# marios2019/CSN

Measured on AMD Instinct MI355X. Metric: CSA fwd+bwd points/sec (10k pts x 256 ch, K=3), higher is better.
Workload: dtype bf16x3 (fp32 operands split into 2 bf16, 3 bf16 MFMA per product, fp32 accumulate); 1 GPU; BASELINE configs[2]: CSA K=3, 32 query shapes/GPU x 10000 pts x 256 ch, n_heads=1, d_k=d_v=256, 20 blocks of 500, 39 classes, fwd + masked CE + bwd, train mode (dropout 0.1 live, 2K+2 evaluations/shape), math mode bf16x3; K=3, parallelism=single GPU

## Files before the change

### csn_amd/_lib.py

```python
from __future__ import annotations

import ctypes
import hashlib
import os
import subprocess
from ctypes import c_char_p, c_double, c_float, c_int, c_longlong, c_ulonglong, c_void_p
from typing import Optional

_HERE = os.path.dirname(os.path.abspath(__file__))
_CSRC = os.path.join(_HERE, "csrc")
LIB_PATH = os.path.join(_HERE, "libcsn_hip.so")
SOURCES = ["gemm_f32.hip", "gemm_bf16x3.hip", "wx_stream.hip", "wx_lnb.hip", "loss.hip", "attn_f32.hip", "attn_bf16x3.hip", "attn_dkv.hip", "attn_dv_scores.hip", "fold.hip", "outproj_ln.hip", "retrieval.hip", "retrieval_screen.hip", "combine.hip", "compat.hip", "minkowski_csn.hip", "minkowski_seg.hip", "rows_fc.hip", "sparse_conv.hip", "sparse_conv_maps16.hip", "train_maps16.hip", "sparse_conv_cat.hip", "octant_conv.hip", "octant_conv_maps16.hip", "octant_conv_stats.hip", "rows_bn_act.hip", "point_field.hip", "kernel_map.hip", "octant_map.hip", "points.hip", "csn_capi.hip"]
HEADERS = ["csn_common.h", "csn_kernels.h", "csn_window.h", "attn_tile_image.h", "wx_common.h", "rows_mma.h", "sconv_gemm_body.inc", "sconv_a16_body.inc", "rows_bn_act_body.inc", "octant_rows_body.inc", os.path.join("..", "..", "include", "csn_hip.h")]
ARCH = "gfx950"
BUILD_FLAGS = [f"--offload-arch={ARCH}", "-O3", "-std=c++17", "-fPIC", "-fvisibility=hidden", "-shared"]

_lib: Optional[ctypes.CDLL] = None


class CsnError(RuntimeError):
    pass


class BnTerms(ctypes.Structure):
# ... 285 lines not shown
    "csn_sparse_conv_stats_fwd_t16": (c_int, [c_void_p, c_int, c_longlong, c_int, c_void_p, c_int, c_int, c_int, c_int, c_void_p, c_void_p,
                                              c_longlong, c_void_p, c_void_p, c_void_p, c_void_p, c_float, c_float, c_void_p,
                                              c_longlong, c_void_p]),
    "csn_rows_bn_act_fwd_t16": (c_int, [c_void_p, c_int, c_int, c_int, c_int, c_float, c_void_p, c_int, c_longlong, c_int, c_void_p,
                                        c_int, c_longlong, c_void_p]),
    "csn_rows_bn_act_bwd_t16": (c_int, [c_void_p, c_longlong, c_void_p, c_int, c_longlong, c_void_p, c_int, c_int, c_int, c_int,
                                        c_float, c_int, c_void_p, c_longlong, c_void_p, c_longlong, c_void_p]),
    "csn_sparse_conv_bwd_t16": (c_int, [c_void_p, c_longlong, c_void_p, c_int, c_longlong, c_int, c_int, c_int, c_int, c_int, c_void_p,
                                        c_void_p, c_void_p, c_void_p, c_longlong, c_void_p, c_void_p, c_void_p, c_longlong, c_void_p]),
    "csn_voxel_mean_f32": (c_int, [c_void_p, c_longlong, c_int, c_void_p, c_void_p, c_int, c_int, c_void_p, c_longlong, c_void_p]),
    "csn_point_interp_fwd_f32": (c_int, [c_void_p, c_longlong, c_int, c_void_p, c_void_p, c_void_p, c_int, c_int, c_void_p, c_longlong,
                                         c_void_p]),
    "csn_point_interp_bwd_f32": (c_int, [c_void_p, c_longlong, c_int, c_void_p, c_void_p, c_void_p, c_void_p, c_int, c_int, c_void_p,
                                         c_longlong, c_void_p]),
    "csn_coord_keys_i64": (c_int, [c_void_p, c_int, c_int, c_void_p, c_void_p, c_void_p]),
    "csn_coord_down_i64": (c_int, [c_void_p, c_int, c_int, c_void_p, c_void_p]),
    "csn_kernel_map_i32": (c_int, [c_void_p, c_void_p, c_int, c_void_p, c_int, c_int, c_int, c_void_p, c_void_p, c_void_p]),
    "csn_octant_partition_i32": (c_int, [c_void_p, c_void_p, c_int, c_int, c_void_p, c_void_p, c_int, c_void_p, c_void_p, c_void_p, c_void_p,
                                         c_void_p]),
    "csn_octant_order_workspace_bytes": (c_longlong, [c_int]),
    "csn_octant_order_i32": (c_int, [c_void_p, c_int, c_void_p, c_void_p, c_void_p, c_longlong, c_void_p, c_void_p]),
    "csn_points_normalize_f32": (c_int, [c_void_p, c_void_p, c_int, c_longlong, c_int, c_void_p, c_void_p, c_void_p]),
    "csn_points_bounds_f64": (c_int, [c_void_p, c_void_p, c_int, c_longlong, c_void_p, c_void_p, c_int, c_void_p, c_void_p, c_void_p]),
    "csn_points_batch_f32": (c_int, [c_void_p, c_void_p, c_void_p, c_int, c_longlong, c_void_p, c_void_p, c_void_p, c_void_p, c_int,
                                     c_int, c_double, c_double, c_double, c_void_p, c_void_p, c_void_p, c_void_p, c_longlong, c_void_p,
                                     c_void_p]),
    "csn_field_index_i32": (c_int, [c_void_p, c_void_p, c_void_p, c_int, c_int, c_void_p, c_void_p, c_void_p, c_void_p, c_void_p,
                                    c_void_p]),
}

EXPORTS = tuple(_SIGNATURES)
DEV_BIG_TILES, DEV_WIDE_GEMM, DEV_WIDE_FORMS, DEV_WX, DEV_LNB_GROUP, DEV_SCONV_NB, DEV_KV_SAME = 0, 1, 2, 3, 5, 7, 8
DEV_ATTN_WG64, DEV_ATTN_WG64_LAUNCHES = 9, 10
DEV_WX_DEFAULT = 9


def lib() -> ctypes.CDLL:
    global _lib
    if _lib is None:
        path = os.environ.get("CSN_LIB_PATH", LIB_PATH)
        if not os.path.exists(path):
            raise CsnError(f"{path} is missing: run `python -c 'import __graft_entry__ as g; g.build()'` "
                           "(there is no CPU or eager fallback for the CSA kernels)")
        handle = ctypes.CDLL(path)
        for name, (res, args) in _SIGNATURES.items():
            fn = getattr(handle, name)
            fn.restype = res
            fn.argtypes = args
        if handle.csn_version() != 17:
            raise CsnError("libcsn_hip.so ABI version mismatch")
        _lib = _Hooked(handle)
    return _lib


_call_hook = None


def set_call_hook(fn) -> None:
    global _call_hook
    _call_hook = fn


class _Hooked:

    def __init__(self, handle):
        self._handle = handle
# ... 24 lines not shown
```

### csn_amd/csrc/csn_capi.hip

```cpp
#include "../../include/csn_hip.h"
#include "csn_kernels.h"
#include <cmath>

namespace {

int g_math_mode = CSN_MATH_BF16X3;
thread_local int t_math_mode = -1;

inline int mode() { return t_math_mode >= 0 ? t_math_mode : g_math_mode; }
thread_local int t_act16 = 0;
inline int act16() { return t_act16 & 3; }
inline bool grad16() { return (t_act16 & 4) != 0; }
inline bool act16_fwd_ok() { return act16() == 0 || (act16() == 1 && mode() == 2) || (act16() == 2 && mode() == 3); }
inline bool act16_bwd_ok() { return act16() == 0 || mode() == 2; }
thread_local int t_rows16 = 0;
inline int rows_mode() { return mode() >= 2 && !t_rows16 ? 1 : mode(); }
thread_local int t_score_layout = 0;
inline int planes_of(int m) { return m == 1 ? 2 : 1; }

struct ModeGuard {
  int saved;
  explicit ModeGuard(int m) : saved(t_math_mode) { t_math_mode = m; }
  ~ModeGuard() { t_math_mode = saved; }
};
// ... 58 lines not shown
  const int n_chunks = (n_points + chunk - 1) / chunk;
  const long long slabs = (long long)n_maps * n_chunks;
  if (ws_floats < slabs * rows * cols) return CSN_E_WORKSPACE;
  CsnGemmArgs g;
  g.A = operand(a, chunk, 0, a_stride, nullptr, lda);
  g.B = operand(b, chunk, 0, b_stride, nullptr, ldb);
  g.A.fmt = a_fmt; g.B.fmt = b_fmt;
  g.C = operand(ws, (long long)rows * cols, 0, (long long)n_chunks * rows * cols, nullptr, cols);
  g.M = rows; g.N = cols; g.K = n_points;
  g.n0 = n_chunks; g.n1 = 1; g.k_chunk = chunk;
  g.alpha = 1.f; g.div_rows = 0; g.div_val = 1.f; g.accumulate = 0; g.eval_ids = nullptr;
  int rc = launch_gemm(g, 1, (int)slabs, st);
  if (rc) return rc;
  return csn_launch_slab_reduce(ws, dw, (int)slabs, (long long)rows * cols, scale, accumulate, st);
}

}

extern "C" {

int csn_version(void) { return CSN_ABI_VERSION; }

int csn_dev_get(int key) {
  switch (key) {
    case CSN_DEV_BIG_TILES: return csn_gemm_big_tiles;
    case CSN_DEV_WIDE_GEMM: return csn_gemm_wide;
    case CSN_DEV_WIDE_FORMS: return csn_gemm_wide_set;
    case CSN_DEV_WX: return csn_dev_wx;
    case CSN_DEV_LNB_GROUP: return csn_dev_lnb_group;
    case CSN_DEV_SCONV_NB: return csn_dev_sconv_nb;
    case CSN_DEV_KV_SAME: return csn_dev_kv_same;
    case CSN_DEV_ATTN_WG64: return csn_dev_attn_wg64;
    case CSN_DEV_ATTN_WG64_LAUNCHES: return csn_dev_attn_wg64_launches;
    default: return CSN_E_ARG;
  }
}
int csn_dev_set(int key, int value) {
  const int prev = csn_dev_get(key);
  switch (key) {
    case CSN_DEV_BIG_TILES: csn_gemm_big_tiles = value; break;
    case CSN_DEV_WIDE_GEMM: csn_gemm_wide = value; break;
    case CSN_DEV_WIDE_FORMS: csn_gemm_wide_set = value; break;
    case CSN_DEV_WX:
      if (value & ~(1 | 4 | 8)) return CSN_E_ARG;
      csn_dev_wx = value;
      break;
    case CSN_DEV_LNB_GROUP: csn_dev_lnb_group = value < 0 ? 0 : value; break;
    case CSN_DEV_SCONV_NB:
      if (value < 0 || value > 4) return CSN_E_ARG;
      csn_dev_sconv_nb = value;
      break;
    case CSN_DEV_KV_SAME:
      if (value != 0 && value != 1) return CSN_E_ARG;
      csn_dev_kv_same = value;
      break;
    case CSN_DEV_ATTN_WG64:
      if (value != 0 && value != 1) return CSN_E_ARG;
      csn_dev_attn_wg64 = value;
      break;
    case CSN_DEV_ATTN_WG64_LAUNCHES: return CSN_E_ARG;
    default: return CSN_E_ARG;
  }
  return prev;
}

int csn_set_math_mode(int m) {
  if (m < 0 || m > 3) return CSN_E_ARG;
  g_math_mode = m;
  return 0;
}
int csn_set_thread_math_mode(int m) {
  if (m < -1 || m > 3) return CSN_E_ARG;
  t_math_mode = m;
  return 0;
}
int csn_get_math_mode(void) { return mode(); }
int csn_get_thread_math_mode(void) { return t_math_mode; }
int csn_set_thread_act16(int fmt) {
  if (fmt < 0 || (fmt & 3) == 3 || fmt > 6 || fmt == 4) return CSN_E_ARG;
  t_act16 = fmt;
  return 0;
}
int csn_get_thread_act16(void) { return t_act16; }
int csn_set_thread_rows16(int on) {
  if (on != 0 && on != 1) return CSN_E_ARG;
  t_rows16 = on;
  return 0;
}
int csn_get_thread_rows16(void) { return t_rows16; }
int csn_set_thread_score_layout(int layout) {
  if (layout < 0 || layout > 1) return CSN_E_ARG;
  t_score_layout = layout;
  return 0;
// ... 73 lines not shown
    if (mis16(x) || mis16(w_qkv) || mis16(q_out) || mis16(kv_out)) return CSN_E_PTR;
    if ((x_shape_stride & 3) || (q_shape_stride & 3) || (kv_shape_stride & 7)) return CSN_E_STRIDE;
    CsnWxArgs a;
    a.w = w_qkv; a.x = x; a.x_item_stride = x_shape_stride; a.ldx = ld_x;
    a.out = kv_out; a.out_item_stride = kv_shape_stride; a.ldo = ld_kv;
    a.out_f32 = q_out; a.out_f32_item_stride = q_shape_stride; a.ldo_f32 = ld_q; a.n_f32 = 1;
    a.n_items = n_shapes; a.n_points = n_points; a.n_sets = 3;
    a.div_rows = d_inner; a.div_val = temperature; a.div_rcp = 1.f / temperature;
    int ex = 0;
    a.div_exact = (std::frexp(temperature, &ex) == 0.5f && temperature > 0.f) ? 1 : 0;
    a.tb = block;
    const int rc = csn_launch_wx(a, 4, (hipStream_t)stream);
    if (rc != CSN_NOT_TAKEN) return rc;
  }
  const int rc = csn_project_f32(x, x_shape_stride, ld_x, w_qkv, d_inner, channels, q_out, q_shape_stride, ld_q, n_shapes, n_points,
                                 d_inner, temperature, 0, 0, stream);
  if (rc) return rc;
  return csn_project_f32(x, x_shape_stride, ld_x, w_qkv + (long long)d_inner * channels, 2 * d_inner, channels,
                         static_cast<float*>(kv_out), kv_shape_stride, ld_kv, n_shapes, n_points, 0, 1.f, 2, block, stream);
}

static int gemm_exact(const float* a, int lda, const float* b, int ldb, int b_is_nk, float* c, int ldc, int M, int N, int K,
                      float div_val, hipStream_t st) {
  CsnGemmArgs g;
  g.A = operand(a, 0, 0, 0, nullptr, lda);
  g.B = operand(b, 0, 0, 0, nullptr, ldb);
  g.C = operand(c, 0, 0, 0, nullptr, ldc);
  g.M = M; g.N = N; g.K = K;
  g.n0 = 1; g.n1 = 1; g.k_chunk = 0;
  g.alpha = 1.f; g.div_rows = div_val != 1.f ? M : 0; g.div_val = div_val; g.accumulate = 0; g.eval_ids = nullptr;
  return csn_launch_gemm_f32(g, b_is_nk, 1, st);
}

long long csn_fold_workspace_floats(int d_inner, int channels) {
  return (d_inner <= 0 || channels <= 0) ? 0 : 2ll * d_inner * channels;
}

int csn_fold_weights_f32(const float* w_q, const float* w_k, const float* w_v, const float* w_fc, int d_inner, int channels,
                         float temperature, float* m, float* w_fv, float* w_fv_t, float* ws, long long ws_floats, void* stream) {
  if (!w_q || !w_k || !w_v || !w_fc || !m || !w_fv || !w_fv_t || !ws || d_inner <= 0 || channels <= 0) return CSN_E_ARG;
  if (!(temperature > 0.f)) return CSN_E_ARG;
  if ((d_inner & 3) || (channels & 3)) return CSN_E_ALIGN;
  if (mis16(w_q) || mis16(w_k) || mis16(w_v) || mis16(w_fc) || mis16(m) || mis16(w_fv) || mis16(w_fv_t) || mis16(ws)) return CSN_E_PTR;
  if (ws_floats < csn_fold_workspace_floats(d_inner, channels)) return CSN_E_WORKSPACE;
  hipStream_t st = (hipStream_t)stream;
  const int D = d_inner, C = channels;
  float* wk_t = ws;
  float* wv_t = ws + (long long)D * C;
  CsnTransposeArgs t;
  t.src[0] = w_k; t.dst[0] = wk_t; t.src[1] = w_v; t.dst[1] = wv_t; t.src[2] = nullptr; t.dst[2] = nullptr;
  t.n = 2; t.rows = D; t.cols = C;
  int rc = csn_launch_transpose_f32(t, st);
  if (rc) return rc;
  rc = gemm_exact(wk_t, D, w_q, C, 0, m, C, C, C, D, temperature, st);
  if (rc) return rc;
  rc = gemm_exact(w_fc, D, w_v, C, 0, w_fv, C, C, C, D, 1.f, st);
  if (rc) return rc;
  return gemm_exact(wv_t, D, w_fc, D, 1, w_fv_t, C, C, C, D, 1.f, st);
}

int csn_unfold_wgrads_f32(const float* dm, const float* dw_fv, const float* w_q, const float* w_k, const float* w_v,
                          const float* w_fc, int d_inner, int channels, float temperature, float* dw_q, float* dw_k, float* dw_v,
                          float* dw_fc, float* ws, long long ws_floats, void* stream) {
  if (!dm || !dw_fv || !w_q || !w_k || !w_v || !w_fc || !dw_q || !dw_k || !dw_v || !dw_fc || !ws || d_inner <= 0 || channels <= 0)
    return CSN_E_ARG;
  if (!(temperature > 0.f)) return CSN_E_ARG;
  if ((d_inner & 3) || (channels & 3)) return CSN_E_ALIGN;
  if (mis16(dm) || mis16(dw_fv) || mis16(w_q) || mis16(w_k) || mis16(w_v) || mis16(w_fc) || mis16(dw_q) || mis16(dw_k) ||
      mis16(dw_v) || mis16(dw_fc) || mis16(ws))
    return CSN_E_PTR;
  if (ws_floats < (long long)d_inner * channels) return CSN_E_WORKSPACE;
  hipStream_t st = (hipStream_t)stream;
  const int D = d_inner, C = channels;
  CsnTransposeArgs t;
  t.src[0] = w_fc; t.dst[0] = ws; t.src[1] = t.src[2] = nullptr; t.dst[1] = t.dst[2] = nullptr;
  t.n = 1; t.rows = C; t.cols = D;
  int rc = csn_launch_transpose_f32(t, st);
  if (rc) return rc;
  rc = gemm_exact(w_k, C, dm, C, 0, dw_q, C, D, C, C, temperature, st);
  if (rc) return rc;
  rc = gemm_exact(w_q, C, dm, C, 1, dw_k, C, D, C, C, temperature, st);
  if (rc) return rc;
  rc = gemm_exact(dw_fv, C, w_v, C, 1, dw_fc, D, C, D, C, 1.f, st);
  if (rc) return rc;
  return gemm_exact(ws, C, dw_fv, C, 0, dw_v, C, D, C, C, 1.f, st);
}

int csn_tile_planes_f32(const float* x, long long x_shape_stride, int ld_x, void* out, long long out_shape_stride, int ld_out,
                        int n_shapes, int rows, int n_points, int block, void* stream) {
  if (!x || !out || n_shapes <= 0 || rows <= 0 || n_points <= 0) return CSN_E_ARG;
  if (block <= 0 || block > 512 || (ld_out % 1024)) return CSN_E_ARG;
  if (((long long)n_points + block - 1) / block * 1024 > ld_out || n_points > ld_x) return CSN_E_ARG;
  if (rows > 65535 || n_shapes > 65535) return CSN_E_ARG;
  if ((block & 3) || (ld_x & 3) || (n_points & 3)) return CSN_E_ALIGN;
  if (mis16(x) || mis16(out)) return CSN_E_PTR;
  if ((x_shape_stride & 3) || (out_shape_stride & 7)) return CSN_E_STRIDE;
  CsnTilePlanesArgs a;
  a.x = x; a.x_item_stride = x_shape_stride; a.ldx = ld_x;
  a.out = static_cast<short*>(out); a.out_item_stride = out_shape_stride; a.ldo = ld_out;
  a.n_items = n_shapes; a.rows = rows; a.n_points = n_points; a.tb = block;
  return csn_launch_tile_planes(a, (hipStream_t)stream);
}

static int attn_fwd_impl(const float* q, const float* k, const float* v, long long q_shape_stride,
                         long long kv_shape_stride, const int* q_index, const int* kv_index, int ld, float* ctx,
                         long long ctx_eval_stride, float* scores, float* lse, int n_evals, int n_heads,
// ... 1678 lines not shown
```

### csn_amd/csrc/csn_kernels.h

```cpp
#pragma once
#include "csn_common.h"

struct CsnGemmArgs {
  CsnOperand A, B, C;
  int M, N, K;
  int n0, n1;
  int k_chunk;
  float alpha;
  int div_rows;
  float div_val;
  int accumulate;
  const int* eval_ids;
  int batch;
  const int* grp_off = nullptr;
  const int* grp_items = nullptr;
  const int* n_arr = nullptr;
  const int* k_arr = nullptr;
  int n_last = 0, k_last = 0;
};

int csn_launch_gemm_f32(const CsnGemmArgs& a, int b_is_nk, int batch, hipStream_t st);
int csn_launch_gemm_bf16x3(const CsnGemmArgs& a, int b_is_nk, int batch, int mode, hipStream_t st);
int csn_gemm_tile_major_planes(int M, int N);
int csn_gemm_bf16x3_big_tiles(int M, int N);
int csn_launch_slab_reduce(const float* slab, float* out, int n_slabs, long long n, float alpha, int accumulate,
                           hipStream_t st);

struct CsnWxArgs {
  const float* w;
  const float* x;  long long x_item_stride;  int ldx;
  void* out;  long long out_item_stride;  int ldo;
  int n_items, n_points, n_sets;
  int div_rows;  float div_val;  float div_rcp;  int div_exact;
  int tb;
  const float* res = nullptr;  long long res_shape_stride = 0;  const int* res_index = nullptr;
  float* rstd = nullptr;
  float eps = 0.f, dropout_p = 0.f;  unsigned long long seed = 0;
  float* sum_ws = nullptr;  int sum_slots = 0;
  float* out_f32 = nullptr;  long long out_f32_item_stride = 0;  int ldo_f32 = 0;  int n_f32 = 0;
};
constexpr int CSN_NOT_TAKEN = -1000;
extern int csn_gemm_big_tiles, csn_gemm_wide, csn_gemm_wide_set, csn_dev_wx, csn_dev_lnb_group;
bool csn_wx_geometry_takes(int n_items, int n_points, int n_sets);
bool csn_wx_takes(int rows, int k);
int csn_launch_wx(const CsnWxArgs& a, int out_mode , hipStream_t st);
int csn_wx_ln_sum_slots(int n_items, int n_points);
int csn_launch_wx_ln_sums(const float* ws, float* out, int n_items, int n_points, hipStream_t st);

struct CsnTilePlanesArgs {
  const float* x;  long long x_item_stride;  int ldx;
  short* out;  long long out_item_stride;  int ldo;
  int n_items, rows, n_points;
  int tb;
};
// ... 382 lines not shown
```

### csn_amd/csrc/gemm_f32.hip

```cpp
#include "csn_common.h"
#include "csn_kernels.h"

namespace {

constexpr int BK = 32;
constexpr int LDS_PAD = 4;
constexpr int LDK = BK + LDS_PAD;

template <int BM, int BN, bool B_NK>
__global__ __launch_bounds__(256, 2) void csn_gemm_f32_kernel(CsnGemmArgs p) {
  constexpr int MT = BM / 64, NT = BN / 64;
  constexpr int A_PASS = BM / 32;
  constexpr int B_PASS = BN / 32;
  constexpr int TPR = BN / 4;
  constexpr int RPP = 256 / TPR;
  constexpr int A_EL = BM * LDK, B_EL = B_NK ? BN * LDK : BK * BN;
  constexpr int STAGE_EL = 4 * 32 * (BN / 2);
  __shared__ __attribute__((aligned(16))) float smem[(A_EL + B_EL) > STAGE_EL ? (A_EL + B_EL) : STAGE_EL];
  float* As = smem;
  float* Bs = smem + A_EL;

  const int tid = threadIdx.x, lane = tid & 63, wave = tid >> 6;
  const int l31 = lane & 31, h = lane >> 5;
  const int wm0 = (wave >> 1) * (BM / 2), wn0 = (wave & 1) * (BN / 2);

  const int tiles_n = (p.N + BN - 1) / BN, tiles = tiles_n * ((p.M + BM - 1) / BM);
  const int L = blockIdx.x, jj = L >> 3;
  const int tile = jj % tiles;
  int z = (jj / tiles) * 8 + (L & 7);
  if (z >= p.batch) return;
  const int tile_m = tile / tiles_n, tile_n = tile % tiles_n;
  const int z0 = z % p.n0; z /= p.n0;
  const int z1 = z % p.n1;
  const int z2 = p.eval_ids ? p.eval_ids[z / p.n1] : z / p.n1;
  const int lda = p.A.ld, ldb = p.B.ld, ldc = p.C.ld;
  const int M = p.M, N = (p.n_last > 0 && z0 == p.n0 - 1) ? p.n_last : (p.n_arr ? ((p.n_arr[z2] + 3) & ~3) : p.N);
  int K = (p.k_last > 0 && z0 == p.n0 - 1) ? p.k_last : (p.k_arr ? p.k_arr[z2] : p.K);
  if (p.k_chunk > 0) { K = min(p.k_chunk, p.K - z0 * p.k_chunk); }
  if (tile_n * BN >= N) return;
  const int m0 = tile_m * BM, n0 = tile_n * BN;

  const csn_rsrc_t Ar = csn_make_rsrc(csn_operand_base(p.A, z0, z1, z2) + (long long)m0 * lda, (long long)BM * lda * 4);
  const csn_rsrc_t Br = B_NK ? csn_make_rsrc(csn_operand_base(p.B, z0, z1, z2) + (long long)n0 * ldb, (long long)BN * ldb * 4)
                             : csn_make_rsrc(csn_operand_base(p.B, z0, z1, z2) + n0, ((long long)(K - 1) * ldb + (N - n0)) * 4);
  const csn_rsrc_t Cr = csn_make_rsrc(csn_operand_base(p.C, z0, z1, z2) + (long long)m0 * ldc + n0, (long long)BM * ldc * 4);

  f32x16 acc[MT][NT];
#pragma unroll
  for (int i = 0; i < MT; ++i)
#pragma unroll
    for (int j = 0; j < NT; ++j)
#pragma unroll
      for (int r = 0; r < 16; ++r) acc[i][j][r] = 0.f;

  const int pr = tid >> 3, pc = (tid & 7) * 4;
  const int kr = tid / TPR, kc = (tid % TPR) * 4;
  unsigned a_off[A_PASS], b_off[B_PASS];
#pragma unroll
  for (int i = 0; i < A_PASS; ++i) a_off[i] = (m0 + pr + 32 * i) < M ? (unsigned)((pr + 32 * i) * lda + pc) * 4u : CSN_OOB;
#pragma unroll
  for (int i = 0; i < B_PASS; ++i) {
    if (B_NK) b_off[i] = (n0 + pr + 32 * i) < N ? (unsigned)((pr + 32 * i) * ldb + pc) * 4u : CSN_OOB;
    else b_off[i] = (n0 + kc) < N ? (unsigned)((kr + RPP * i) * ldb + kc) * 4u : CSN_OOB;
  }

  f32x4 ra[A_PASS], rb[B_PASS];
  auto load_slab = [&](int k0) {
    const unsigned kp = (k0 + pc) < K ? 0u : CSN_OOB;
#pragma unroll
    for (int i = 0; i < A_PASS; ++i) ra[i] = csn_bload4(Ar, a_off[i] | kp, (unsigned)k0 * 4u);
    if (B_NK) {
#pragma unroll
      for (int i = 0; i < B_PASS; ++i) rb[i] = csn_bload4(Br, b_off[i] | kp, (unsigned)k0 * 4u);
    } else {
#pragma unroll
      for (int i = 0; i < B_PASS; ++i) {
        const unsigned kq = (k0 + kr + RPP * i) < K ? 0u : CSN_OOB;
        rb[i] = csn_bload4(Br, b_off[i] | kq, (unsigned)k0 * (unsigned)ldb * 4u);
      }
    }
  };
  auto store_slab = [&]() {
#pragma unroll
    for (int i = 0; i < A_PASS; ++i) *reinterpret_cast<f32x4*>(&As[(pr + 32 * i) * LDK + pc]) = ra[i];
    if (B_NK) {
#pragma unroll
      for (int i = 0; i < B_PASS; ++i) *reinterpret_cast<f32x4*>(&Bs[(pr + 32 * i) * LDK + pc]) = rb[i];
    } else {
#pragma unroll
      for (int i = 0; i < B_PASS; ++i) *reinterpret_cast<f32x4*>(&Bs[(kr + RPP * i) * BN + kc]) = rb[i];
    }
  };

  const int nk = (K + BK - 1) / BK;
  if (nk > 0) { load_slab(0); store_slab(); }
  __syncthreads();
  for (int kt = 0; kt < nk; ++kt) {
    if (kt + 1 < nk) load_slab((kt + 1) * BK);
#pragma unroll
    for (int kk = 0; kk < BK; kk += 8) {
      f32x4 af[MT], bf[NT];
#pragma unroll
      for (int i = 0; i < MT; ++i)
        af[i] = *reinterpret_cast<const f32x4*>(&As[(wm0 + 32 * i + l31) * LDK + kk + 4 * h]);
#pragma unroll
      for (int j = 0; j < NT; ++j) {
        if (B_NK) {
          bf[j] = *reinterpret_cast<const f32x4*>(&Bs[(wn0 + 32 * j + l31) * LDK + kk + 4 * h]);
        } else {
#pragma unroll
          for (int t = 0; t < 4; ++t) bf[j][t] = Bs[(kk + 4 * h + t) * BN + wn0 + 32 * j + l31];
        }
      }
#pragma unroll
      for (int t = 0; t < 4; ++t)
#pragma unroll
        for (int i = 0; i < MT; ++i)
#pragma unroll
          for (int j = 0; j < NT; ++j) acc[i][j] = csn_mfma(af[i][t], bf[j][t], acc[i][j]);
    }
    __syncthreads();
    if (kt + 1 < nk) { store_slab(); __syncthreads(); }
  }

  const float alpha = p.alpha;
  constexpr int WN = BN / 2;
  constexpr int CPR = WN / 4;
  constexpr int RPI = 64 / CPR;
  constexpr int NCH = 32 / RPI;
  float* wbuf = smem + wave * 32 * WN;
  const int cc = lane % CPR, rsub = lane / CPR;
  const int col = wn0 + 4 * cc;
  const bool n_ok = (n0 + col) < N;
#pragma unroll
  for (int i = 0; i < MT; ++i) {
#pragma unroll
    for (int j = 0; j < NT; ++j)
#pragma unroll
      for (int r = 0; r < 16; ++r) {
        float v = acc[i][j][r] * alpha;
        if ((m0 + wm0 + 32 * i + csn_acc_row(r, h)) < p.div_rows) v = v / p.div_val;
        wbuf[csn_acc_row(r, h) * WN + 32 * j + l31] = v;
      }
    f32x4 vals[NCH];
    unsigned off[NCH];
#pragma unroll
    for (int t = 0; t < NCH; ++t) {
      const int row = RPI * t + rsub;
      vals[t] = *reinterpret_cast<const f32x4*>(&wbuf[row * WN + 4 * cc]);
      const int ml = wm0 + 32 * i + row;
      off[t] = (n_ok && (m0 + ml) < M) ? (unsigned)(ml * ldc + col) * 4u : CSN_OOB;
    }
    if (p.accumulate) {
      f32x4 prev[NCH];
#pragma unroll
      for (int t = 0; t < NCH; ++t) prev[t] = csn_bload4(Cr, off[t]);
#pragma unroll
      for (int t = 0; t < NCH; ++t) vals[t] += prev[t];
    }
#pragma unroll
    for (int t = 0; t < NCH; ++t) csn_bstore4(vals[t], Cr, off[t]);
  }
}

__global__ __launch_bounds__(256) void csn_slab_reduce_kernel(const float* __restrict__ slab, float* __restrict__ out,
                                                              int n_slabs, long long n, float alpha, int accumulate) {
  const long long i = ((long long)blockIdx.x * blockDim.x + threadIdx.x) * 4;
  if (i >= n) return;
  if (i + 3 < n && (n & 3) == 0) {
    f32x4 s0 = {0.f, 0.f, 0.f, 0.f}, s1 = s0, s2 = s0, s3 = s0;
    int z = 0;
    for (; z + 3 < n_slabs; z += 4) {
      s0 += *reinterpret_cast<const f32x4*>(slab + (long long)z * n + i);
      s1 += *reinterpret_cast<const f32x4*>(slab + (long long)(z + 1) * n + i);
      s2 += *reinterpret_cast<const f32x4*>(slab + (long long)(z + 2) * n + i);
      s3 += *reinterpret_cast<const f32x4*>(slab + (long long)(z + 3) * n + i);
    }
    for (; z < n_slabs; ++z) s0 += *reinterpret_cast<const f32x4*>(slab + (long long)z * n + i);
    f32x4 s = ((s0 + s1) + (s2 + s3)) * alpha;
    if (accumulate) s += *reinterpret_cast<const f32x4*>(out + i);
    *reinterpret_cast<f32x4*>(out + i) = s;
  } else {
    const long long end = i + 4 < n ? i + 4 : n;
    for (long long j = i; j < end; ++j) {
      float s = 0.f;
      for (int z = 0; z < n_slabs; ++z) s += slab[(long long)z * n + j];
      s *= alpha;
      if (accumulate) s += out[j];
      out[j] = s;
    }
  }
}

}

template <int BM, int BN, bool B_NK>
static int launch(const CsnGemmArgs& a, int batch, hipStream_t st) {
  CsnGemmArgs b = a;
  b.batch = batch;
  const long long tiles = (long long)((a.N + BN - 1) / BN) * ((a.M + BM - 1) / BM);
  dim3 grid((unsigned)(((batch + 7) / 8) * 8 * tiles));
  hipLaunchKernelGGL((csn_gemm_f32_kernel<BM, BN, B_NK>), grid, dim3(256), 0, st, b);
  return (int)hipGetLastError();
}

int csn_launch_gemm_f32(const CsnGemmArgs& a, int b_is_nk, int batch, hipStream_t st) {
  if (a.M <= 0 || a.N <= 0 || batch <= 0) return 0;
  if ((a.A.ld & 3) || (a.B.ld & 3) || (a.K & 3) || (a.k_chunk & 3)) return -2;
  if (a.N & 3) return -2;
  if ((reinterpret_cast<uintptr_t>(a.A.ptr) & 15) || (reinterpret_cast<uintptr_t>(a.B.ptr) & 15)) return -3;
  if ((a.A.s0 & 3) || (a.A.s1 & 3) || (a.A.s2 & 3) || (a.B.s0 & 3) || (a.B.s1 & 3) || (a.B.s2 & 3)) return -4;
  if (a.M <= 64) return b_is_nk ? launch<64, 128, true>(a, batch, st) : launch<64, 128, false>(a, batch, st);
  return b_is_nk ? launch<128, 128, true>(a, batch, st) : launch<128, 128, false>(a, batch, st);
}

int csn_launch_slab_reduce(const float* slab, float* out, int n_slabs, long long n, float alpha, int accumulate,
                           hipStream_t st) {
  if (n <= 0) return 0;
  hipLaunchKernelGGL(csn_slab_reduce_kernel, dim3((unsigned)((n + 255) / 256)), dim3(64), 0, st, slab, out, n_slabs, n,
                     alpha, accumulate);
  return (int)hipGetLastError();
}
```

### include/csn_hip.h

```cpp
#ifndef CSN_HIP_H
#define CSN_HIP_H

#ifdef __cplusplus
extern "C" {
#endif

#define CSN_ABI_VERSION 17
#define CSN_API __attribute__((visibility("default")))

#define CSN_MATH_FP32 0
#define CSN_MATH_BF16X3 1
#define CSN_MATH_BF16 2
#define CSN_MATH_FP16 3

#define CSN_E_ARG (-1)
#define CSN_E_ALIGN (-2)
#define CSN_E_PTR (-3)
#define CSN_E_STRIDE (-4)
#define CSN_E_DIM (-5)
#define CSN_E_WORKSPACE (-6)

CSN_API int csn_version(void);
CSN_API int csn_set_thread_act16(int fmt);
CSN_API int csn_get_thread_act16(void);
// ... 337 lines not shown
typedef struct CsnCatParts {
  const float* x[4];
  long long ld_x[4];
  int c_in[4];
} CsnCatParts;
CSN_API long long csn_sparse_conv_cat_stats_workspace_bytes(int n_out, int c_out);
CSN_API int csn_sparse_conv_cat_stats_fwd_f32(const CsnCatParts* parts, int n_parts, int n_in, const int* table, int n_out, int kv,
                                      int c_out, const float* w, float* z, long long ld_z, float* mean, float* invstd,
                                      float* running_mean, float* running_var, float eps, float momentum, void* ws,
                                      long long ws_bytes, void* stream);

CSN_API int csn_sparse_conv_stats_fwd_t16(const void* x, int x16, long long ld_x, int n_in, const int* table, int n_out, int kv, int c_in,
                                  int c_out, const float* w, float* z, long long ld_z, float* mean, float* invstd,
                                  float* running_mean, float* running_var, float eps, float momentum, void* ws, long long ws_bytes,
                                  void* stream);
CSN_API int csn_rows_bn_act_fwd_t16(const CsnBnTerms* terms, int n_terms, int n_rows, int channels, int training, float eps,
                            const void* r, int r16, long long ld_r, int relu, void* y, int y16, long long ld_y, void* stream);
CSN_API int csn_rows_bn_act_bwd_t16(const float* dy, long long ld_dy, const void* y, int y16, long long ld_y, const CsnBnTerms* terms,
                            int n_terms, int n_rows, int channels, int training, float eps, int relu, float* dr, long long ld_dr,
                            void* ws, long long ws_bytes, void* stream);
CSN_API int csn_sparse_conv_bwd_t16(const float* dy, long long ld_dy, const void* x, int x16, long long ld_x, int n_in, int n_out, int kv,
                            int c_in, int c_out, const int* fwd_table, const int* bwd_table, const float* w, float* dx,
                            long long ld_dx, float* dw, float* dbias, void* ws, long long ws_bytes, void* stream);

#define CSN_DEV_BIG_TILES 0
#define CSN_DEV_WIDE_GEMM 1
#define CSN_DEV_WIDE_FORMS 2
#define CSN_DEV_WX 3
#define CSN_DEV_LNB_GROUP 5
#define CSN_DEV_SCONV_NB 7
#define CSN_DEV_KV_SAME 8
#define CSN_DEV_ATTN_WG64 9
#define CSN_DEV_ATTN_WG64_LAUNCHES 10
CSN_API int csn_dev_set(int key, int value);
CSN_API int csn_dev_get(int key);

#ifdef __cplusplus
}
#endif
#endif
```

Before: 18.62 million points/s.

## Batch weight-fold GEMMs into one grouped launch with transposed-A loads

Adds a grouped fp32 GEMM kernel that takes a table of up to four independent problems and runs them in a single launch, indexing the problem through blockIdx.z. The shared tile body gains support for a K-major A operand, so the fold forward and backward paths no longer need explicit transpose kernels and workspace copies before their GEMMs. This is meant to remove several small launches and transpose passes on the weight-fold path, which is enabled by default. In exchange the tiles are a fixed 64x64 and blocks whose problem has fewer tiles than the largest one exit early.

Result: no change. 18.65 million points/s, median of 6 (+0.2%).

```diff
diff --git a/csn_amd/_lib.py b/csn_amd/_lib.py
--- a/csn_amd/_lib.py
+++ b/csn_amd/_lib.py
@@ -341,6 +341,7 @@
 EXPORTS = tuple(_SIGNATURES)
 DEV_BIG_TILES, DEV_WIDE_GEMM, DEV_WIDE_FORMS, DEV_WX, DEV_LNB_GROUP, DEV_SCONV_NB, DEV_KV_SAME = 0, 1, 2, 3, 5, 7, 8
 DEV_ATTN_WG64, DEV_ATTN_WG64_LAUNCHES = 9, 10
+DEV_GEMM_TABLE = 11
 DEV_WX_DEFAULT = 9
 
 
diff --git a/csn_amd/csrc/csn_capi.hip b/csn_amd/csrc/csn_capi.hip
--- a/csn_amd/csrc/csn_capi.hip
+++ b/csn_amd/csrc/csn_capi.hip
@@ -114,6 +114,7 @@
     case CSN_DEV_KV_SAME: return csn_dev_kv_same;
     case CSN_DEV_ATTN_WG64: return csn_dev_attn_wg64;
     case CSN_DEV_ATTN_WG64_LAUNCHES: return csn_dev_attn_wg64_launches;
+    case CSN_DEV_GEMM_TABLE: return csn_dev_gemm_table;
     default: return CSN_E_ARG;
   }
 }
@@ -141,6 +142,10 @@
       csn_dev_attn_wg64 = value;
       break;
     case CSN_DEV_ATTN_WG64_LAUNCHES: return CSN_E_ARG;
+    case CSN_DEV_GEMM_TABLE:
+      if (value != 0 && value != 1) return CSN_E_ARG;
+      csn_dev_gemm_table = value;
+      break;
     default: return CSN_E_ARG;
   }
   return prev;
@@ -280,6 +285,14 @@
   return csn_launch_gemm_f32(g, b_is_nk, 1, st);
 }
 
+static CsnGemmProblem problem(const float* a, int lda, int a_km, const float* b, int ldb, int b_nk, float* c, int ldc, int M, int N,
+                              int K, float div_val) {
+  CsnGemmProblem q;
+  q.a = a; q.b = b; q.c = c; q.lda = lda; q.ldb = ldb; q.ldc = ldc; q.M = M; q.N = N; q.K = K; q.a_km = a_km; q.b_nk = b_nk;
+  q.div_val = div_val;
+  return q;
+}
+
 long long csn_fold_workspace_floats(int d_inner, int channels) {
   return (d_inner <= 0 || channels <= 0) ? 0 : 2ll * d_inner * channels;
 }
@@ -293,6 +306,14 @@
   if (ws_floats < csn_fold_workspace_floats(d_inner, channels)) return CSN_E_WORKSPACE;
   hipStream_t st = (hipStream_t)stream;
   const int D = d_inner, C = channels;
+  if (csn_dev_gemm_table) {
+    CsnGemmTable g;
+    g.n = 3;
+    g.p[0] = problem(w_k, C, 1, w_q, C, 0, m, C, C, C, D, temperature);
+    g.p[1] = problem(w_fc, D, 0, w_v, C, 0, w_fv, C, C, C, D, 1.f);
+    g.p[2] = problem(w_v, C, 1, w_fc, D, 1, w_fv_t, C, C, C, D, 1.f);
+    return csn_launch_gemm_f32_table(g, st);
+  }
   float* wk_t = ws;
   float* wv_t = ws + (long long)D * C;
   CsnTransposeArgs t;
@@ -320,6 +341,15 @@
   if (ws_floats < (long long)d_inner * channels) return CSN_E_WORKSPACE;
   hipStream_t st = (hipStream_t)stream;
   const int D = d_inner, C = channels;
+  if (csn_dev_gemm_table) {
+    CsnGemmTable g;
+    g.n = 4;
+    g.p[0] = problem(w_k, C, 0, dm, C, 0, dw_q, C, D, C, C, temperature);
+    g.p[1] = problem(w_q, C, 0, dm, C, 1, dw_k, C, D, C, C, temperature);
+    g.p[2] = problem(dw_fv, C, 0, w_v, C, 1, dw_fc, D, C, D, C, 1.f);
+    g.p[3] = problem(w_fc, D, 1, dw_fv, C, 0, dw_v, C, D, C, C, 1.f);
+    return csn_launch_gemm_f32_table(g, st);
+  }
   CsnTransposeArgs t;
   t.src[0] = w_fc; t.dst[0] = ws; t.src[1] = t.src[2] = nullptr; t.dst[1] = t.dst[2] = nullptr;
   t.n = 1; t.rows = C; t.cols = D;
diff --git a/csn_amd/csrc/csn_kernels.h b/csn_amd/csrc/csn_kernels.h
--- a/csn_amd/csrc/csn_kernels.h
+++ b/csn_amd/csrc/csn_kernels.h
@@ -20,6 +20,18 @@
 };
 
 int csn_launch_gemm_f32(const CsnGemmArgs& a, int b_is_nk, int batch, hipStream_t st);
+constexpr int CSN_GEMM_TABLE_MAX = 4;
+struct CsnGemmProblem {
+  const float* a;  const float* b;  float* c;
+  int lda, ldb, ldc, M, N, K, a_km, b_nk;
+  float div_val;
+};
+struct CsnGemmTable {
+  CsnGemmProblem p[CSN_GEMM_TABLE_MAX];
+  int n;
+};
+int csn_launch_gemm_f32_table(const CsnGemmTable& t, hipStream_t st);
+extern int csn_dev_gemm_table;
 int csn_launch_gemm_bf16x3(const CsnGemmArgs& a, int b_is_nk, int batch, int mode, hipStream_t st);
 int csn_gemm_tile_major_planes(int M, int N);
 int csn_gemm_bf16x3_big_tiles(int M, int N);
diff --git a/csn_amd/csrc/gemm_f32.hip b/csn_amd/csrc/gemm_f32.hip
--- a/csn_amd/csrc/gemm_f32.hip
+++ b/csn_amd/csrc/gemm_f32.hip
@@ -6,17 +6,23 @@
 constexpr int BK = 32;
 constexpr int LDS_PAD = 4;
 constexpr int LDK = BK + LDS_PAD;
-
-template <int BM, int BN, bool B_NK>
-__global__ __launch_bounds__(256, 2) void csn_gemm_f32_kernel(CsnGemmArgs p) {
+constexpr int gemm_a_el(int bm, bool a_km) { return a_km ? BK * bm : bm * LDK; }
+constexpr int gemm_b_el(int bn, bool b_nk) { return b_nk ? bn * LDK : BK * bn; }
+constexpr int gemm_smem_el(int bm, int bn, bool b_nk, bool a_km) {
+  const int slabs = gemm_a_el(bm, a_km) + gemm_b_el(bn, b_nk), stage = 4 * 32 * (bn / 2);
+  return slabs > stage ? slabs : stage;
+}
+
+template <int BM, int BN, bool B_NK, bool A_KM>
+CSN_DEVINL void csn_gemm_f32_tile(float* smem, const float* a_base, const float* b_base, float* c_base, int lda, int ldb, int ldc,
+                                  int M, int N, int K, int m0, int n0, float alpha, int div_rows, float div_val, int accumulate) {
   constexpr int MT = BM / 64, NT = BN / 64;
   constexpr int A_PASS = BM / 32;
   constexpr int B_PASS = BN / 32;
   constexpr int TPR = BN / 4;
   constexpr int RPP = 256 / TPR;
-  constexpr int A_EL = BM * LDK, B_EL = B_NK ? BN * LDK : BK * BN;
-  constexpr int STAGE_EL = 4 * 32 * (BN / 2);
-  __shared__ __attribute__((aligned(16))) float smem[(A_EL + B_EL) > STAGE_EL ? (A_EL + B_EL) : STAGE_EL];
+  constexpr int A_TPR = BM / 4, A_RPP = 256 / A_TPR;
+  constexpr int A_EL = gemm_a_el(BM, A_KM);
   float* As = smem;
   float* Bs = smem + A_EL;
 
@@ -24,6 +30,152 @@
   const int l31 = lane & 31, h = lane >> 5;
   const int wm0 = (wave >> 1) * (BM / 2), wn0 = (wave & 1) * (BN / 2);
 
+  const csn_rsrc_t Ar = A_KM ? csn_make_rsrc(a_base + m0, ((long long)(K - 1) * lda + (M - m0)) * 4)
+                             : csn_make_rsrc(a_base + (long long)m0 * lda, (long long)BM * lda * 4);
+  const csn_rsrc_t Br = B_NK ? csn_make_rsrc(b_base + (long long)n0 * ldb, (long long)BN * ldb * 4)
+                             : csn_make_rsrc(b_base + n0, ((long long)(K - 1) * ldb + (N - n0)) * 4);
+  const csn_rsrc_t Cr = csn_make_rsrc(c_base + (long long)m0 * ldc + n0, (long long)BM * ldc * 4);
+
+  f32x16 acc[MT][NT];
+#pragma unroll
+  for (int i = 0; i < MT; ++i)
+#pragma unroll
+    for (int j = 0; j < NT; ++j)
+#pragma unroll
+      for (int r = 0; r < 16; ++r) acc[i][j][r] = 0.f;
+
+  const int pr = tid >> 3, pc = (tid & 7) * 4;
+  const int kr = tid / TPR, kc = (tid % TPR) * 4;
+  const int akr = tid / A_TPR, akc = (tid % A_TPR) * 4;
+  unsigned a_off[A_PASS], b_off[B_PASS];
+#pragma unroll
+  for (int i = 0; i < A_PASS; ++i) {
+    if (A_KM) a_off[i] = (m0 + akc) < M ? (unsigned)((akr + A_RPP * i) * lda + akc) * 4u : CSN_OOB;
+    else a_off[i] = (m0 + pr + 32 * i) < M ? (unsigned)((pr + 32 * i) * lda + pc) * 4u : CSN_OOB;
+  }
+#pragma unroll
+  for (int i = 0; i < B_PASS; ++i) {
+    if (B_NK) b_off[i] = (n0 + pr + 32 * i) < N ? (unsigned)((pr + 32 * i) * ldb + pc) * 4u : CSN_OOB;
+    else b_off[i] = (n0 + kc) < N ? (unsigned)((kr + RPP * i) * ldb + kc) * 4u : CSN_OOB;
+  }
+
+  f32x4 ra[A_PASS], rb[B_PASS];
+  auto load_slab = [&](int k0) {
+    const unsigned kp = (k0 + pc) < K ? 0u : CSN_OOB;
+#pragma unroll
+    for (int i = 0; i < A_PASS; ++i) {
+      if (A_KM) {
+        const unsigned kq = (k0 + akr + A_RPP * i) < K ? 0u : CSN_OOB;
+        ra[i] = csn_bload4(Ar, a_off[i] | kq, (unsigned)k0 * (unsigned)lda * 4u);
+      } else {
+        ra[i] = csn_bload4(Ar, a_off[i] | kp, (unsigned)k0 * 4u);
+      }
+    }
+    if (B_NK) {
+#pragma unroll
+      for (int i = 0; i < B_PASS; ++i) rb[i] = csn_bload4(Br, b_off[i] | kp, (unsigned)k0 * 4u);
+    } else {
+#pragma unroll
+      for (int i = 0; i < B_PASS; ++i) {
+        const unsigned kq = (k0 + kr + RPP * i) < K ? 0u : CSN_OOB;
+        rb[i] = csn_bload4(Br, b_off[i] | kq, (unsigned)k0 * (unsigned)ldb * 4u);
+      }
+    }
+  };
+  auto store_slab = [&]() {
+#pragma unroll
+    for (int i = 0; i < A_PASS; ++i) {
+      if (A_KM) *reinterpret_cast<f32x4*>(&As[(akr + A_RPP * i) * BM + akc]) = ra[i];
+      else *reinterpret_cast<f32x4*>(&As[(pr + 32 * i) * LDK + pc]) = ra[i];
+    }
+    if (B_NK) {
+#pragma unroll
+      for (int i = 0; i < B_PASS; ++i) *reinterpret_cast<f32x4*>(&Bs[(pr + 32 * i) * LDK + pc]) = rb[i];
+    } else {
+#pragma unroll
+      for (int i = 0; i < B_PASS; ++i) *reinterpret_cast<f32x4*>(&Bs[(kr + RPP * i) * BN + kc]) = rb[i];
+    }
+  };
+
+  const int nk = (K + BK - 1) / BK;
+  if (nk > 0) { load_slab(0); store_slab(); }
+  __syncthreads();
+  for (int kt = 0; kt < nk; ++kt) {
+    if (kt + 1 < nk) load_slab((kt + 1) * BK);
+#pragma unroll
+    for (int kk = 0; kk < BK; kk += 8) {
+      f32x4 af[MT], bf[NT];
+#pragma unroll
+      for (int i = 0; i < MT; ++i) {
+        if (A_KM) {
+#pragma unroll
+          for (int t = 0; t < 4; ++t) af[i][t] = As[(kk + 4 * h + t) * BM + wm0 + 32 * i + l31];
+        } else {
+          af[i] = *reinterpret_cast<const f32x4*>(&As[(wm0 + 32 * i + l31) * LDK + kk + 4 * h]);
+        }
+      }
+#pragma unroll
+      for (int j = 0; j < NT; ++j) {
+        if (B_NK) {
+          bf[j] = *reinterpret_cast<const f32x4*>(&Bs[(wn0 + 32 * j + l31) * LDK + kk + 4 * h]);
+        } else {
+#pragma unroll
+          for (int t = 0; t < 4; ++t) bf[j][t] = Bs[(kk + 4 * h + t) * BN + wn0 + 32 * j + l31];
+        }
+      }
+#pragma unroll
+      for (int t = 0; t < 4; ++t)
+#pragma unroll
+        for (int i = 0; i < MT; ++i)
+#pragma unroll
+          for (int j = 0; j < NT; ++j) acc[i][j] = csn_mfma(af[i][t], bf[j][t], acc[i][j]);
+    }
+    __syncthreads();
+    if (kt + 1 < nk) { store_slab(); __syncthreads(); }
+  }
+
+  constexpr int WN = BN / 2;
+  constexpr int CPR = WN / 4;
+  constexpr int RPI = 64 / CPR;
+  constexpr int NCH = 32 / RPI;
+  float* wbuf = smem + wave * 32 * WN;
+  const int cc = lane % CPR, rsub = lane / CPR;
+  const int col = wn0 + 4 * cc;
+  const bool n_ok = (n0 + col) < N;
+#pragma unroll
+  for (int i = 0; i < MT; ++i) {
+#pragma unroll
+    for (int j = 0; j < NT; ++j)
+#pragma unroll
+      for (int r = 0; r < 16; ++r) {
+        float v = acc[i][j][r] * alpha;
+        if ((m0 + wm0 + 32 * i + csn_acc_row(r, h)) < div_rows) v = v / div_val;
+        wbuf[csn_acc_row(r, h) * WN + 32 * j + l31] = v;
+      }
+    f32x4 vals[NCH];
+    unsigned off[NCH];
+#pragma unroll
+    for (int t = 0; t < NCH; ++t) {
+      const int row = RPI * t + rsub;
+      vals[t] = *reinterpret_cast<const f32x4*>(&wbuf[row * WN + 4 * cc]);
+      const int ml = wm0 + 32 * i + row;
+      off[t] = (n_ok && (m0 + ml) < M) ? (unsigned)(ml * ldc + col) * 4u : CSN_OOB;
+    }
+    if (accumulate) {
+      f32x4 prev[NCH];
+#pragma unroll
+      for (int t = 0; t < NCH; ++t) prev[t] = csn_bload4(Cr, off[t]);
+#pragma unroll
+      for (int t = 0; t < NCH; ++t) vals[t] += prev[t];
+    }
+#pragma unroll
+    for (int t = 0; t < NCH; ++t) csn_bstore4(vals[t], Cr, off[t]);
+  }
+}
+
+template <int BM, int BN, bool B_NK>
+__global__ __launch_bounds__(256, 2) void csn_gemm_f32_kernel(CsnGemmArgs p) {
+  __shared__ __attribute__((aligned(16))) float smem[gemm_smem_el(BM, BN, B_NK, false)];
   const int tiles_n = (p.N + BN - 1) / BN, tiles = tiles_n * ((p.M + BM - 1) / BM);
   const int L = blockIdx.x, jj = L >> 3;
   const int tile = jj % tiles;
@@ -33,134 +185,29 @@
   const int z0 = z % p.n0; z /= p.n0;
   const int z1 = z % p.n1;
   const int z2 = p.eval_ids ? p.eval_ids[z / p.n1] : z / p.n1;
-  const int lda = p.A.ld, ldb = p.B.ld, ldc = p.C.ld;
-  const int M = p.M, N = (p.n_last > 0 && z0 == p.n0 - 1) ? p.n_last : (p.n_arr ? ((p.n_arr[z2] + 3) & ~3) : p.N);
+  const int N = (p.n_last > 0 && z0 == p.n0 - 1) ? p.n_last : (p.n_arr ? ((p.n_arr[z2] + 3) & ~3) : p.N);
   int K = (p.k_last > 0 && z0 == p.n0 - 1) ? p.k_last : (p.k_arr ? p.k_arr[z2] : p.K);
   if (p.k_chunk > 0) { K = min(p.k_chunk, p.K - z0 * p.k_chunk); }
   if (tile_n * BN >= N) return;
-  const int m0 = tile_m * BM, n0 = tile_n * BN;
-
-  const csn_rsrc_t Ar = csn_make_rsrc(csn_operand_base(p.A, z0, z1, z2) + (long long)m0 * lda, (long long)BM * lda * 4);
-  const csn_rsrc_t Br = B_NK ? csn_make_rsrc(csn_operand_base(p.B, z0, z1, z2) + (long long)n0 * ldb, (long long)BN * ldb * 4)
-                             : csn_make_rsrc(csn_operand_base(p.B, z0, z1, z2) + n0, ((long long)(K - 1) * ldb + (N - n0)) * 4);
-  const csn_rsrc_t Cr = csn_make_rsrc(csn_operand_base(p.C, z0, z1, z2) + (long long)m0 * ldc + n0, (long long)BM * ldc * 4);
-
-  f32x16 acc[MT][NT];
-#pragma unroll
-  for (int i = 0; i < MT; ++i)
-#pragma unroll
-    for (int j = 0; j < NT; ++j)
-#pragma unroll
-      for (int r = 0; r < 16; ++r) acc[i][j][r] = 0.f;
-
-  const int pr = tid >> 3, pc = (tid & 7) * 4;
-  const int kr = tid / TPR, kc = (tid % TPR) * 4;
-  unsigned a_off[A_PASS], b_off[B_PASS];
-#pragma unroll
-  for (int i = 0; i < A_PASS; ++i) a_off[i] = (m0 + pr + 32 * i) < M ? (unsigned)((pr + 32 * i) * lda + pc) * 4u : CSN_OOB;
-#pragma unroll
-  for (int i = 0; i < B_PASS; ++i) {
-    if (B_NK) b_off[i] = (n0 + pr + 32 * i) < N ? (unsigned)((pr + 32 * i) * ldb + pc) * 4u : CSN_OOB;
-    else b_off[i] = (n0 + kc) < N ? (unsigned)((kr + RPP * i) * ldb + kc) * 4u : CSN_OOB;
-  }
-
-  f32x4 ra[A_PASS], rb[B_PASS];
-  auto load_slab = [&](int k0) {
-    const unsigned kp = (k0 + pc) < K ? 0u : CSN_OOB;
-#pragma unroll
-    for (int i = 0; i < A_PASS; ++i) ra[i] = csn_bload4(Ar, a_off[i] | kp, (unsigned)k0 * 4u);
-    if (B_NK) {
-#pragma unroll
-      for (int i = 0; i < B_PASS; ++i) rb[i] = csn_bload4(Br, b_off[i] | kp, (unsigned)k0 * 4u);
-    } else {
-#pragma unroll
-      for (int i = 0; i < B_PASS; ++i) {
-        const unsigned kq = (k0 + kr + RPP * i) < K ? 0u : CSN_OOB;
-        rb[i] = csn_bload4(Br, b_off[i] | kq, (unsigned)k0 * (unsigned)ldb * 4u);
-      }
-    }
-  };
-  auto store_slab = [&]() {
-#pragma unroll
-    for (int i = 0; i < A_PASS; ++i) *reinterpret_cast<f32x4*>(&As[(pr + 32 * i) * LDK + pc]) = ra[i];
-    if (B_NK) {
-#pragma unroll
-      for (int i = 0; i < B_PASS; ++i) *reinterpret_cast<f32x4*>(&Bs[(pr + 32 * i) * LDK + pc]) = rb[i];
-    } else {
-#pragma unroll
-      for (int i = 0; i < B_PASS; ++i) *reinterpret_cast<f32x4*>(&Bs[(kr + RPP * i) * BN + kc]) = rb[i];
-    }
-  };
-
-  const int nk = (K + BK - 1) / BK;
-  if (nk > 0) { load_slab(0); store_slab(); }
-  __syncthreads();
-  for (int kt = 0; kt < nk; ++kt) {
-    if (kt + 1 < nk) load_slab((kt + 1) * BK);
-#pragma unroll
-    for (int kk = 0; kk < BK; kk += 8) {
-      f32x4 af[MT], bf[NT];
-#pragma unroll
-      for (int i = 0; i < MT; ++i)
-        af[i] = *reinterpret_cast<const f32x4*>(&As[(wm0 + 32 * i + l31) * LDK + kk + 4 * h]);
-#pragma unroll
-      for (int j = 0; j < NT; ++j) {
-        if (B_NK) {
-          bf[j] = *reinterpret_cast<const f32x4*>(&Bs[(wn0 + 32 * j + l31) * LDK + kk + 4 * h]);
-        } else {
-#pragma unroll
-          for (int t = 0; t < 4; ++t) bf[j][t] = Bs[(kk + 4 * h + t) * BN + wn0 + 32 * j + l31];
-        }
-      }
-#pragma unroll
-      for (int t = 0; t < 4; ++t)
-#pragma unroll
-        for (int i = 0; i < MT; ++i)
-#pragma unroll
-          for (int j = 0; j < NT; ++j) acc[i][j] = csn_mfma(af[i][t], bf[j][t], acc[i][j]);
-    }
-    __syncthreads();
-    if (kt + 1 < nk) { store_slab(); __syncthreads(); }
-  }
-
-  const float alpha = p.alpha;
-  constexpr int WN = BN / 2;
-  constexpr int CPR = WN / 4;
-  constexpr int RPI = 64 / CPR;
-  constexpr int NCH = 32 / RPI;
-  float* wbuf = smem + wave * 32 * WN;
-  const int cc = lane % CPR, rsub = lane / CPR;
-  const int col = wn0 + 4 * cc;
-  const bool n_ok = (n0 + col) < N;
-#pragma unroll
-  for (int i = 0; i < MT; ++i) {
-#pragma unroll
-    for (int j = 0; j < NT; ++j)
-#pragma unroll
-      for (int r = 0; r < 16; ++r) {
-        float v = acc[i][j][r] * alpha;
-        if ((m0 + wm0 + 32 * i + csn_acc_row(r, h)) < p.div_rows) v = v / p.div_val;
-        wbuf[csn_acc_row(r, h) * WN + 32 * j + l31] = v;
-      }
-    f32x4 vals[NCH];
-    unsigned off[NCH];
-#pragma unroll
-    for (int t = 0; t < NCH; ++t) {
-      const int row = RPI * t + rsub;
-      vals[t] = *reinterpret_cast<const f32x4*>(&wbuf[row * WN + 4 * cc]);
-      const int ml = wm0 + 32 * i + row;
-      off[t] = (n_ok && (m0 + ml) < M) ? (unsigned)(ml * ldc + col) * 4u : CSN_OOB;
-    }
-    if (p.accumulate) {
-      f32x4 prev[NCH];
-#pragma unroll
-      for (int t = 0; t < NCH; ++t) prev[t] = csn_bload4(Cr, off[t]);
-#pragma unroll
-      for (int t = 0; t < NCH; ++t) vals[t] += prev[t];
-    }
-#pragma unroll
-    for (int t = 0; t < NCH; ++t) csn_bstore4(vals[t], Cr, off[t]);
-  }
+  csn_gemm_f32_tile<BM, BN, B_NK, false>(smem, csn_operand_base(p.A, z0, z1, z2), csn_operand_base(p.B, z0, z1, z2),
+                                         csn_operand_base(p.C, z0, z1, z2), p.A.ld, p.B.ld, p.C.ld, p.M, N, K, tile_m * BM,
+                                         tile_n * BN, p.alpha, p.div_rows, p.div_val, p.accumulate);
+}
+
+template <int BM, int BN>
+__global__ __launch_bounds__(256, 2) void csn_gemm_f32_table_kernel(CsnGemmTable t) {
+  __shared__ __attribute__((aligned(16))) float smem[gemm_smem_el(BM, BN, true, false)];
+  static_assert(gemm_smem_el(BM, BN, true, false) >= gemm_smem_el(BM, BN, false, true), "LDS of the table kernel");
+  const CsnGemmProblem& q = t.p[blockIdx.z];
+  const int tiles_n = (q.N + BN - 1) / BN;
+  const int m0 = (int)(blockIdx.x / tiles_n) * BM, n0 = (int)(blockIdx.x % tiles_n) * BN;
+  if (m0 >= q.M) return;
+  const int div_rows = q.div_val != 1.f ? q.M : 0;
+#define CSN_TABLE_TILE(B_NK, A_KM) \
+  csn_gemm_f32_tile<BM, BN, B_NK, A_KM>(smem, q.a, q.b, q.c, q.lda, q.ldb, q.ldc, q.M, q.N, q.K, m0, n0, 1.f, div_rows, q.div_val, 0)
+  if (q.a_km) { if (q.b_nk) CSN_TABLE_TILE(true, true); else CSN_TABLE_TILE(false, true); }
+  else        { if (q.b_nk) CSN_TABLE_TILE(true, false); else CSN_TABLE_TILE(false, false); }
+#undef CSN_TABLE_TILE
 }
 
 __global__ __launch_bounds__(256) void csn_slab_reduce_kernel(const float* __restrict__ slab, float* __restrict__ out,
@@ -214,6 +261,25 @@
   return b_is_nk ? launch<128, 128, true>(a, batch, st) : launch<128, 128, false>(a, batch, st);
 }
 
+int csn_dev_gemm_table = 1;
+
+int csn_launch_gemm_f32_table(const CsnGemmTable& t, hipStream_t st) {
+  constexpr int BT = 64;
+  if (t.n <= 0 || t.n > CSN_GEMM_TABLE_MAX) return -1;
+  int tiles = 0;
+  for (int i = 0; i < t.n; ++i) {
+    const CsnGemmProblem& q = t.p[i];
+    if (q.M <= 0 || q.N <= 0 || q.K <= 0) return -1;
+    if ((q.lda & 3) || (q.ldb & 3) || (q.ldc & 3) || (q.K & 3) || (q.N & 3) || (q.a_km && (q.M & 3))) return -2;
+    if ((reinterpret_cast<uintptr_t>(q.a) & 15) || (reinterpret_cast<uintptr_t>(q.b) & 15) || (reinterpret_cast<uintptr_t>(q.c) & 15))
+      return -3;
+    const int ti = ((q.M + BT - 1) / BT) * ((q.N + BT - 1) / BT);
+    tiles = ti > tiles ? ti : tiles;
+  }
+  hipLaunchKernelGGL((csn_gemm_f32_table_kernel<BT, BT>), dim3((unsigned)tiles, 1, (unsigned)t.n), dim3(256), 0, st, t);
+  return (int)hipGetLastError();
+}
+
 int csn_launch_slab_reduce(const float* slab, float* out, int n_slabs, long long n, float alpha, int accumulate,
                            hipStream_t st) {
   if (n <= 0) return 0;
diff --git a/include/csn_hip.h b/include/csn_hip.h
--- a/include/csn_hip.h
+++ b/include/csn_hip.h
@@ -393,6 +393,7 @@
 #define CSN_DEV_KV_SAME 8
 #define CSN_DEV_ATTN_WG64 9
 #define CSN_DEV_ATTN_WG64_LAUNCHES 10
+#define CSN_DEV_GEMM_TABLE 11
 CSN_API int csn_dev_set(int key, int value);
 CSN_API int csn_dev_get(int key);
 
```
